# ShiLab-Bioinformatics/subread

Hardware: AMD Instinct MI355X
Metric: Mreads/s aligned, 100bp SE vs 3Gbp index; 1/2/4/8-GPU scaling + HBM GB/s (higher is better)
Workload: dtype u32; 1 GPU; C3: 50M x 100bp SE reads vs 3.0 Gbp 24-contig genome, full one-block index; read_len=100, mode=subread-align SE, parallelism=reads sharded across 1 GPU(s), index replicated, no collective

## Files before the change

### subread_amd/csrc/svg_device.h

```cpp
#ifndef SVG_DEVICE_H
#define SVG_DEVICE_H
#include <hip/hip_runtime.h>
#include <stdint.h>
#include "subread_vote.h"
#include "svg_internal.h"

struct DevIndex {
	const uint32_t *bstart;
	const int16_t *keys;
	const uint32_t *vals;
	const uint8_t *values;
	const uint32_t *chr_end;
	uint32_t nb, n_chr;
	uint32_t start_point, length, start_base_offset, values_bytes;
	int32_t gap, padding;
	const uint32_t *bgrp;
	const uint8_t *keys8;
	const uint4 *bline;
	const uint4 *bcode;
	const uint32_t *khash;
	const uint32_t *khash_ff;
	uint64_t khash_lines;
	int32_t khash_sec;
	const uint32_t *ksorted;
// ... 130 lines not shown
	return 0;
}

int svg_index_finish_device(svg_index *h);

static inline int svg_ensure(svg_index *h, void **p, size_t *cap, size_t need)
{
	if (need <= *cap) return 0;
	hipFree(*p);
	*p = NULL;
	*cap = 0;
	if (dmalloc(h, p, need)) return SVG_E_NOMEM;
	*cap = need;
	return 0;
}

void svg_io_free(svg_index *h);
void svg_long_ws_free(svg_index *h);

struct KParams {
	svg_params p;
	DevIndex ix;
	const char *seq1, *seq2;
	const uint64_t *off1, *off2;
	const uint16_t *len1, *len2;
	uint64_t n_reads;
	uint8_t *out;
	uint8_t *jout;
	uint16_t *bm_out;
	uint32_t *scratch;
	unsigned long long *stats;
	int tol, ii_end;
	uint32_t low, high;
	const uint2 *precs;
	int nps;
	uint32_t prec_stride;
	const uint32_t *idx;
	const uint32_t *idx_count;
	uint32_t *work;
	int32_t static_eighths;
	int stored;
	uint32_t *err;
};

struct PParams {
	DevIndex ix;
	const char *seq1, *seq2;
	const uint64_t *off1, *off2;
	const uint16_t *len1, *len2;
	uint32_t n_reads;
	int nps;
	int total_subreads, reverse_r1, reverse_r2;
	uint64_t nb_magic;
	uint2 *out;
	int soa;
	int window;
	int readmajor;
	unsigned long long *stats;
	uint32_t group;
	uint32_t *big_list, *big_count;
	uint32_t big_stride, big_regions;
	int packed;
	const uint32_t *pk_bases[2], *pk_xmask[2];
	const uint64_t *pk_starts[2];
	uint64_t pk_stride[2], pk_base0[2];
};

struct VoteJob {
	KParams kp;
	PParams pp;
	int npmax, nps, ends;
	bool sj, lane, overlap_mode;
	uint64_t per_read, chunk;
};
int svg_vote_prepare(svg_index *h, const svg_params *p, const svg_reads *r1, const svg_reads *r2, svg_mapping_result *out,
                     svg_subjunc_result *jout, uint16_t *big_margin, VoteJob *job);
int svg_vote_chunk(svg_index *h, VoteJob *job, uint64_t c0, uint64_t cn, int slot, hipStream_t st, hipStream_t st2);
int svg_vote_chunk_probe(svg_index *h, VoteJob *job, uint64_t c0, uint64_t cn, int slot, hipStream_t st);
int svg_vote_chunk_vote(svg_index *h, VoteJob *job, uint64_t c0, uint64_t cn, int slot, hipStream_t st, hipStream_t st2);
int svg_vote_batch_device_packed(svg_index *h, const svg_params *p, const svg_reads *r1, const svg_reads *r2,
                                 const svg_packed_reads *pk, svg_mapping_result *out, svg_subjunc_result *jout,
                                 uint16_t *big_margin, hipStream_t stream);

int svg_lane_eligible(const svg_index *h, const svg_params *p, int paired, int sj);
int svg_check_params(const svg_index *h, const svg_params *p, int paired);
int svg_lane_chunk(svg_index *h, int slot, const svg_params *p, const uint16_t *len, uint32_t n, const uint2 *precs,
                   int nps, uint8_t *out, uint8_t *jout, uint16_t *bm, const char *seq, const uint64_t *off,
                   unsigned long long *stats, uint32_t **defer_list, uint32_t **defer_count, hipStream_t st);
int svg_lane_pe_chunk(svg_index *h, int slot, const svg_params *p, const uint16_t *len1, const uint16_t *len2, uint32_t n,
                      const uint2 *precs, int nps, uint8_t *out, uint8_t *jout, uint16_t *bm_out, const char *seq1,
                      const uint64_t *off1, const char *seq2, const uint64_t *off2, unsigned long long *stats,
                      uint32_t **defer_list, uint32_t **defer_count, hipStream_t st);
int svg_timing_mark(svg_index *h, int k, int phase, hipStream_t st);

#endif
```

### subread_amd/csrc/svg_vote.hip

```cpp
#include <hip/hip_runtime.h>
#include <string>
#include <vector>
#include <chrono>
#include <atomic>
#include <deque>
#include <condition_variable>
#include <mutex>
#include <thread>
#include <pthread.h>
#include <sys/mman.h>
#include <stdint.h>
#include <string.h>
#include <stdlib.h>
#include <stdio.h>
#include "subread_vote.h"
#include "svg_internal.h"
#include "svg_device.h"

#define ROWS 30
#define SPACE 24
#define PSTR 25
#define NSLOT (ROWS * PSTR)
#define REC_LEN 21
#define COLD_WORDS 8
#define JCW 17

#define CAND_CAP 64
template <int ENDS, int MAXL, int MAXP, bool SJ>
struct WaveLDS {
	static constexpr int MAXS = ENDS == 1 ? 16 : 64;
	static constexpr int CAPL = ENDS == 2 ? 64 : 1;
	uint2 pm[NSLOT];
	uint2 cl[CAPL];
	uint16_t cls[CAPL];
	uint32_t pmid[ENDS][2][MAXP];
	uint16_t pfwd[ENDS][2][MAXP];
	uint16_t pbwd[ENDS][2][MAXP];
	uint32_t pcum[MAXP + 1];
	uint32_t res[ENDS][3][17];
	uint32_t tmp[ENDS][3][17];
	uint32_t jres[SJ ? ENDS : 1][3][4];
	uint32_t jtmp[SJ ? ENDS : 1][3][4];
	uint32_t simp_pos[ENDS][MAXS];
	uint16_t simp_slot[ENDS][MAXS];
	uint16_t simp_votes[ENDS][MAXS];
	int32_t simp_loc[ENDS == 2 ? 2 : 1][ENDS == 2 ? MAXS : 1];
	int16_t simp_chr[ENDS == 2 ? 2 : 1][ENDS == 2 ? MAXS : 1];
	uint16_t bm[SJ ? ENDS : 1][10];
	uint8_t rnew[32];
	alignas(16) unsigned long long btab[32];
	uint8_t gwin[SJ ? 2 : 1][SJ ? 64 : 4];
	char text[SJ ? ENDS : 1][2][SJ ? MAXL : 4];
};

__device__ __forceinline__ int lane_id() { return __lane_id(); }
__device__ __forceinline__ unsigned long long ballot(bool p) { return __ballot(p); }
__device__ __forceinline__ int lanes_below(unsigned long long m) { return __popcll(m & ((1ull << lane_id()) - 1ull)); }
__device__ __forceinline__ void wsync() { __builtin_amdgcn_fence(__ATOMIC_SEQ_CST, "wavefront"); __builtin_amdgcn_wave_barrier(); }
__device__ __forceinline__ int wave_max(int v)
{
	for (int o = 32; o; o >>= 1) { int t = __shfl_xor(v, o); v = t > v ? t : v; }
	return v;
}
__device__ __forceinline__ int wave_min(int v)
{
	for (int o = 32; o; o >>= 1) { int t = __shfl_xor(v, o); v = t < v ? t : v; }
	return v;
}
__device__ __forceinline__ uint32_t wave_sum(uint32_t v)
{
// ... 1296 lines not shown
	};
	auto uni = [](uint64_t v) -> uint64_t {
		return (uint64_t)(uint32_t)__builtin_amdgcn_readfirstlane((int)(uint32_t)v) |
		       ((uint64_t)(uint32_t)__builtin_amdgcn_readfirstlane((int)(uint32_t)(v >> 32)) << 32);
	};
	auto dyn_after = [&](uint64_t p) { return kp.idx && p + nw >= n_static; };
	uint64_t i = !kp.idx || gw < n_static ? gw : (n ? grab() : n);
	uint64_t in = i >= n ? n : (dyn_after(i) ? grab() : i + nw);
	uint64_t r = uni(i < n ? (kp.idx ? kp.idx[i] : i) : 0);
	if (i < n) { W.prefetch_text(r); W.prefetch_recs(r); }
	while (i < n) {
		const bool dyn = in < n && dyn_after(in);
		uint32_t nxt = 0;
		if (dyn && lane_id() == 0) nxt = atomicAdd(kp.work, 1u);
		const uint64_t rn = uni(in < n ? (kp.idx ? kp.idx[in] : in) : kp.n_reads);
		W.run_read(r, rn);
		const uint64_t in2 = in >= n ? n : (dyn ? n_static + (uint64_t)(uint32_t)__builtin_amdgcn_readfirstlane(__shfl((int)nxt, 0)) : in + nw);
		i = in;
		r = rn;
		in = in2;
#ifdef SVG_STAMPS
		{ unsigned long long _t = __builtin_amdgcn_s_memtime(); W.acc[5] += _t - W.t_last; W.t_last = _t; }
#endif
	}
#ifdef SVG_STAMPS
	if (kp.stats && lane_id() == 0) {
		for (int k = 0; k < 8; k++) atomicAdd(&kp.stats[8 + k], W.acc[k]);
		for (int k = 8; k < 12; k++) atomicAdd(&kp.stats[21 + k - 8], W.acc[k]);
		for (int k = 0; k < 4; k++) atomicAdd(&kp.stats[28 + k], W.why[k]);
	}
#endif
}

__device__ __forceinline__ bool try_run(uint64_t eq, int n, int &m, int &fwd, int &bwd, bool &hit)
{
	const int fe = eq ? __builtin_ctzll(eq) : 0, ne = __popcll(eq);
	if (eq && eq != (((ne == 64 ? 0ull : (1ull << ne)) - 1ull) << fe)) return false;
	if (eq) {
		const int le = fe + ne - 1;
		int lo = 0, hi = n - 1;
		for (;;) {
			m = (lo + hi) >> 1;
			if (m < fe) lo = m + 1;
			else if (m > le) hi = m - 1;
			else break;
		}
		hit = true;
		fwd = le - m + 1;
		bwd = m - fe;
	}
	return true;
}

template <int ENDS, bool PACKED>
__device__ __forceinline__ bool probe_key(const PParams &pp, uint32_t r, int e, int s, int p, uint32_t &key)
{
	int len = e ? pp.len2[r] : pp.len1[r];
	if (len > SVG_READ_KEEP) len = SVG_READ_KEEP;
	const int gap = pp.ix.gap;
	if (len < 15 + gap) return false;
	const int cr = (len - 15 - gap) << 16;
	int step;
	if (len <= 160) { step = cr / (pp.total_subreads - 1); if (step < (gap << 16)) step = gap << 16; }
	else { step = 6 << 16; if (cr / step > 62) step = cr / 62; }
	const int np = (1 + cr / step) * gap;
	if (p >= np) return false;
	const int k = p / gap, x = p - k * gap;
	int off = (int)(((int64_t)step * k) >> 16);
	if (gap > 1) off -= off % gap - x;
	const int rev = e ? pp.reverse_r2 : pp.reverse_r1;
	const bool direct = s == rev;
	const int start = direct ? off : len - 16 - off;
	key = 0;
	if constexpr (PACKED) {
		const uint64_t k0 = (pp.pk_starts[e] ? pp.pk_starts[e][r] : pp.pk_base0[e] + (uint64_t)r * pp.pk_stride[e]) +
		                    (uint64_t)start;
		const uint32_t *bw = pp.pk_bases[e] + (k0 >> 4);
		const uint32_t s2 = 2u * (uint32_t)(k0 & 15u);
		const uint32_t W = s2 ? (bw[0] << s2) | (bw[1] >> (32u - s2)) : bw[0];
		uint32_t X2 = 0;
		if (pp.pk_xmask[e]) {
			const uint32_t *xw = pp.pk_xmask[e] + (k0 >> 5);
			const uint32_t s1 = (uint32_t)(k0 & 31u);
			uint32_t t = (s1 > 16u ? (xw[0] << s1) | (xw[1] >> (32u - s1)) : xw[0] << s1) >> 16;
			t = (t | (t << 8)) & 0x00ff00ffu;
			t = (t | (t << 4)) & 0x0f0f0f0fu;
			t = (t | (t << 2)) & 0x33333333u;
			t = (t | (t << 1)) & 0x55555555u;
			X2 = t | (t << 1);
		}
		if (direct) key = (s == 1 && rev) ? (W | X2) : W;
		else {
			const uint32_t v = __builtin_bitreverse32(~W | X2);
			key = ((v >> 1) & 0x55555555u) | ((v & 0x55555555u) << 1);
		}
	} else {
		const char *src = (e ? pp.seq2 : pp.seq1) + (e ? pp.off2[r] : pp.off1[r]) + start;
		const uintptr_t a = (uintptr_t)src;
		const uint32_t *w = (const uint32_t *)(a & ~(uintptr_t)3);
		const int sh = (int)(a & 3);
		uint32_t wd[5];
#pragma unroll
		for (int q = 0; q < 4; q++) wd[q] = w[q];
		wd[4] = sh ? w[4] : 0u;
#pragma unroll
		for (int i = 0; i < 16; i++) {
			const int bi = sh + (direct ? i : 15 - i);
			char c = (char)((wd[bi >> 2] >> (8 * (bi & 3))) & 0xff);
			if (!direct) c = comp(c);
			if (s == 1 && rev) c = comp(comp(c));
			key |= b2i(c) << (30 - 2 * i);
		}
	}
	return true;
}

template <int ENDS, int BPC, bool LINE, bool PACKED>
__global__ void __launch_bounds__(256, BPC) probe_kernel(PParams pp)
{
	const DevIndex &ix = pp.ix;
	const uint32_t nps = (uint32_t)pp.nps, per_read = ENDS * 2 * nps;
	const uint32_t total = pp.n_reads * per_read;
	const int gap = ix.gap;
	unsigned long long st_p = 0, st_i = 0, st_h = 0;
	const uint32_t tiles = (total + 255u) / 256u, per_blk = (tiles + gridDim.x - 1u) / gridDim.x;
	const uint32_t tile_end = min(tiles, (blockIdx.x + 1u) * per_blk);
	for (uint32_t tile = blockIdx.x * per_blk; tile < tile_end; tile++) {
		const uint32_t t = tile * 256u + threadIdx.x;
		if (t >= total) break;
		uint32_t r, rem;
		if (pp.soa && !pp.readmajor) { rem = t / pp.n_reads; r = t - rem * pp.n_reads; }
		else { r = t / per_read; rem = t - r * per_read; }
		const int e = ENDS == 2 ? (int)(rem / (2 * nps)) : 0;
		const uint32_t rem2 = rem - (uint32_t)e * 2 * nps;
		const int s = rem2 >= nps ? 1 : 0;
		const int p = (int)(rem2 - (uint32_t)s * nps);
		uint2 rec = make_uint2(0u, 0u);
		uint32_t key;
		if (probe_key<ENDS, PACKED>(pp, r, e, s, p, key)) {
			{
				const uint32_t q = (uint32_t)__umul64hi((uint64_t)key, pp.nb_magic);
				const uint32_t b = key - q * ix.nb;
				const int16_t k16 = (int16_t)q;
				uint32_t first;
				int n;
				bool compact = false, inl = false;
				uint4 lw[4];
				if constexpr (LINE) {
					const uint4 *l4 = ix.bline + 4 * (size_t)b;
#pragma unroll
					for (int q = 0; q < 4; q++) lw[q] = l4[q];
					const uint32_t c = lw[0].y & 255u;
					first = lw[0].x;
					n = (int)c;
					compact = c != 255u;
					inl = c <= 59u;
				} else if (ix.bgrp) {
					const uint4 *g4 = (const uint4 *)(ix.bgrp + 8 * (size_t)(b >> 4));
					const uint4 ga = g4[0], gb = g4[1];
					const uint32_t i = b & 15u;
					const uint32_t cw[4] = {ga.y, ga.z, ga.w, gb.x};
					uint32_t pre = 0;
					bool sat = false;
#pragma unroll
					for (int q = 0; q < 4; q++) {
						const int nb_ = (int)i - 4 * q;
// ... 71 lines not shown
								const uint32_t x = dw[q] ^ kk;
								const uint32_t z = ~(((x & 0x7fff7fffu) + 0x7fff7fffu) | x | 0x7fff7fffu);
								const int j = 4 * k + q;
								eq |= ((uint64_t)((z >> 15) & 1u) << (2 * j)) | ((uint64_t)(z >> 31) << (2 * j + 1));
							}
						}
						eq = (eq >> sh) & ((1ull << n) - 1ull);
						done = try_run(eq, n, m, fwd, bwd, hit);
					}
					if (!done) {
						int lo = 0, hi = n - 1;
						for (;;) {
							m = (lo + hi) >> 1;
							int16_t kk = K[m];
							if (kk > k16) hi = m - 1;
							else if (kk < k16) lo = m + 1;
							else { hit = true; break; }
							if (hi < lo) break;
						}
						if (hit) {
							int qq = m + 1;
							while (qq < n && K[qq] == k16) qq++;
							fwd = qq - m;
							qq = m - 1;
							while (qq >= 0 && K[qq] == k16) qq--;
							bwd = m - 1 - qq;
						}
					}
					if (hit) {
						rec = make_uint2(first + (uint32_t)m, (uint32_t)fwd | ((uint32_t)bwd << 16));
						st_h += (unsigned)(fwd + bwd);
					}
				}
			}
		}
		pp.out[pp.soa ? (size_t)rem * pp.n_reads + r : (size_t)t] = rec;
	}
	if (pp.stats) {
		for (int o = 32; o; o >>= 1) {
			st_p += __shfl_xor(st_p, o); st_i += __shfl_xor(st_i, o); st_h += __shfl_xor(st_h, o);
		}
		if (lane_id() == 0 && st_p) {
			atomicAdd(&pp.stats[0], st_p);
			atomicAdd(&pp.stats[1], st_i);
			atomicAdd(&pp.stats[2], st_h);
		}
	}
}

#define PROBE_GROUP_RECS 2048
#define IMG_LINE  0
#define IMG_CODE  1
#define IMG_KHASH 2
template <int ENDS, bool PACKED>
struct ProbeDepth { static constexpr int value = 2; };

__device__ __forceinline__ void code_record(const uint4 u0, const uint4 u1, uint32_t q, uint32_t key, uint2 &rec, bool &big,
                                            unsigned long long &st_i, unsigned long long &st_h)
{
	const uint32_t c = u0.y & 255u, first = u0.x;
	big = c == 255u;
	if (!big && c) {
		const uint64_t z[4] = {~(((uint64_t)u0.y << 32) | u0.x) & ~0xffffffffffull, ~(((uint64_t)u0.w << 32) | u0.z),
		                       ~(((uint64_t)u1.y << 32) | u1.x), ~(((uint64_t)u1.w << 32) | u1.z)};
		const int k = (int)q;
		const int fe = k ? code_zero(z, k - 1) - 40 - (k - 1) : 0;
		const int ee = code_zero(z, k) - 40 - k;
		st_i += c;
		if (ee > fe) {
			const int le = ee - 1;
			int lo = 0, hi = (int)c - 1, m;
			for (;;) {
				m = (lo + hi) >> 1;
				if (m < fe) lo = m + 1;
				else if (m > le) hi = m - 1;
				else break;
			}
			rec = make_uint2(first + (uint32_t)m, (uint32_t)(le - m + 1) | ((uint32_t)(m - fe) << 16));
			st_h += (unsigned)(ee - fe);
		}
	}
	if (big) rec = make_uint2(key, 0xffffffffu);
}

template <int ENDS, bool PACKED, int IMG>
__global__ void __launch_bounds__(256, 8) probe_line_kernel(PParams pp)
{
	__shared__ uint2 srec[PROBE_GROUP_RECS];
	__shared__ uint32_t s_big;
	const DevIndex &ix = pp.ix;
	const uint32_t nps = (uint32_t)pp.nps, per_read = ENDS * 2 * nps, n = pp.n_reads, G = pp.group;
	const uint32_t ngroups = (n + G - 1) / G, per_blk = (ngroups + gridDim.x - 1) / gridDim.x;
	const uint32_t g_end = min(ngroups, (blockIdx.x + 1) * per_blk);
	uint32_t *const big_list = pp.big_list + (size_t)blockIdx.x * pp.big_stride;
	unsigned long long st_p = 0, st_i = 0, st_h = 0;
	if (threadIdx.x == 0) s_big = 0;
	__syncthreads();
	for (uint32_t g = blockIdx.x * per_blk; g < g_end; g++) {
		const uint32_t r0 = g * G, nr = min(G, n - r0), np = nr * per_read, npr = (np + 255u) & ~255u;
		if constexpr (IMG == IMG_CODE) for (uint32_t i0 = threadIdx.x; i0 < npr; i0 += 256u * ProbeDepth<ENDS, PACKED>::value) {
			uint32_t key[ProbeDepth<ENDS, PACKED>::value], outidx[ProbeDepth<ENDS, PACKED>::value], q[ProbeDepth<ENDS, PACKED>::value];
			bool ok[ProbeDepth<ENDS, PACKED>::value];
#pragma unroll
			for (int t = 0; t < ProbeDepth<ENDS, PACKED>::value; t++) {
				const uint32_t i = i0 + 256u * (uint32_t)t;
				key[t] = outidx[t] = q[t] = 0u;
				ok[t] = false;
				if (i < np) {
					const uint32_t rl = i / per_read, rem = i - rl * per_read, r = r0 + rl;
					const int e = ENDS == 2 ? (int)(rem / (2 * nps)) : 0;
					const uint32_t rem2 = rem - (uint32_t)e * 2 * nps;
					const int s = rem2 >= nps ? 1 : 0;
					const int p = (int)(rem2 - (uint32_t)s * nps);
					outidx[t] = pp.soa ? rem * n + r : r * per_read + rem;
					ok[t] = probe_key<ENDS, PACKED>(pp, r, e, s, p, key[t]);
				}
			}
			uint4 u0[ProbeDepth<ENDS, PACKED>::value], u1[ProbeDepth<ENDS, PACKED>::value];
#pragma unroll
			for (int t = 0; t < ProbeDepth<ENDS, PACKED>::value; t++) {
				u0[t] = u1[t] = make_uint4(0u, 0u, 0u, 0u);
				if (ok[t]) {
					q[t] = (uint32_t)__umul64hi((uint64_t)key[t], pp.nb_magic);
					const uint4 *c4 = ix.bcode + 2 * (size_t)(key[t] - q[t] * ix.nb);
					u0[t] = c4[0];
					u1[t] = c4[1];
				}
			}
#pragma unroll
			for (int t = 0; t < ProbeDepth<ENDS, PACKED>::value; t++) {
				const uint32_t i = i0 + 256u * (uint32_t)t;
				if (i - threadIdx.x >= npr) break;
				uint2 rec = make_uint2(0u, 0u);
				bool big = false;
				if (ok[t]) {
					st_p++;
					code_record(u0[t], u1[t], q[t], key[t], rec, big, st_i, st_h);
				}
				const unsigned long long bm = ballot(big);
				if (bm) {
					const int leader = __ffsll((long long)bm) - 1;
					uint32_t base = 0;
					if (lane_id() == leader) base = atomicAdd(&s_big, (uint32_t)__popcll(bm));
					base = __shfl(base, leader);
					if (big) big_list[base + lanes_below(bm)] = outidx[t];
				}
				if (i < np) srec[i] = rec;
			}
		}
		if (IMG == IMG_KHASH && ix.khash_sec) for (uint32_t i0 = threadIdx.x; i0 < npr; i0 += 256u * ProbeDepth<ENDS, PACKED>::value) {
			uint32_t key[ProbeDepth<ENDS, PACKED>::value], outidx[ProbeDepth<ENDS, PACKED>::value];
			uint64_t L[ProbeDepth<ENDS, PACKED>::value];
			bool ok[ProbeDepth<ENDS, PACKED>::value];
#pragma unroll
			for (int t = 0; t < ProbeDepth<ENDS, PACKED>::value; t++) {
				const uint32_t i = i0 + 256u * (uint32_t)t;
				key[t] = outidx[t] = 0u;
				L[t] = 0u;
				ok[t] = false;
				if (i < np) {
					const uint32_t rl = i / per_read, rem = i - rl * per_read, r = r0 + rl;
					const int e = ENDS == 2 ? (int)(rem / (2 * nps)) : 0;
					const uint32_t rem2 = rem - (uint32_t)e * 2 * nps;
					const int s = rem2 >= nps ? 1 : 0;
					const int p = (int)(rem2 - (uint32_t)s * nps);
					outidx[t] = pp.soa ? rem * n + r : r * per_read + rem;
					ok[t] = probe_key<ENDS, PACKED>(pp, r, e, s, p, key[t]);
				}
			}
			uint4 a[ProbeDepth<ENDS, PACKED>::value], b4[ProbeDepth<ENDS, PACKED>::value];
#pragma unroll
			for (int t = 0; t < ProbeDepth<ENDS, PACKED>::value; t++) {
				a[t] = b4[t] = make_uint4(0u, 0u, 0u, 0u);
				if (ok[t] && key[t] != 0xffffffffu) {
					L[t] = khash_line(key[t], ix.khash_lines);
					const uint4 *l4 = (const uint4 *)(ix.khash + 8 * L[t]);
					a[t] = l4[0];
					b4[t] = l4[1];
				}
			}
#pragma unroll
			for (int t = 0; t < ProbeDepth<ENDS, PACKED>::value; t++) {
				const uint32_t i = i0 + 256u * (uint32_t)t;
				if (i - threadIdx.x >= npr) break;
				uint2 rec = make_uint2(0u, 0u);
				if (ok[t]) {
					st_p++;
					if (pp.stats) {
						const uint32_t q = (uint32_t)__umul64hi((uint64_t)key[t], pp.nb_magic), b = key[t] - q * ix.nb;
						st_i += ix.bstart[b + 1] - ix.bstart[b];
					}
					if (key[t] == 0xffffffffu) khash_find(ix, key[t], rec);
					else {
						bool more;
						if (!khash_sector(a[t], b4[t], key[t], rec, more) && more)
							khash_find_from(ix, key[t], L[t] + 1 == ix.khash_lines ? 0 : L[t] + 1, rec);
					}
					if (pp.stats) st_h += (rec.y & 0xffffu) + (rec.y >> 16);
				}
				if (i < np) srec[i] = rec;
			}
		}
		if (IMG != IMG_CODE && !(IMG == IMG_KHASH && ix.khash_sec)) for (uint32_t i = threadIdx.x; i < npr; i += 256u) {
			uint2 rec = make_uint2(0u, 0u);
			bool big = false;
			uint32_t outidx = 0;
			if (i < np) {
				const uint32_t rl = i / per_read, rem = i - rl * per_read, r = r0 + rl;
				const int e = ENDS == 2 ? (int)(rem / (2 * nps)) : 0;
				const uint32_t rem2 = rem - (uint32_t)e * 2 * nps;
				const int s = rem2 >= nps ? 1 : 0;
				const int p = (int)(rem2 - (uint32_t)s * nps);
				outidx = pp.soa ? rem * n + r : r * per_read + rem;
				uint32_t key;
				if (IMG == IMG_KHASH && probe_key<ENDS, PACKED>(pp, r, e, s, p, key)) {
					st_p++;
					if (pp.stats) {
						const uint32_t q = (uint32_t)__umul64hi((uint64_t)key, pp.nb_magic), b = key - q * ix.nb;
						st_i += ix.bstart[b + 1] - ix.bstart[b];
					}
					khash_find(ix, key, rec);
					if (pp.stats) st_h += (rec.y & 0xffffu) + (rec.y >> 16);
				} else if (IMG == IMG_LINE && probe_key<ENDS, PACKED>(pp, r, e, s, p, key)) {
					const uint32_t q = (uint32_t)__umul64hi((uint64_t)key, pp.nb_magic);
					const uint32_t b = key - q * ix.nb;
					const uint4 *l4 = ix.bline + 4 * (size_t)b;
					uint4 lw[4];
#pragma unroll
					for (int k = 0; k < 4; k++) lw[k] = l4[k];
					const uint32_t c = lw[0].y & 255u, first = lw[0].x;
					st_p++;
					big = c > 59u;
					if (!big && c) {
						const uint32_t kk = (uint32_t)(uint8_t)q * 0x01010101u;
						uint64_t eq = 0;
#pragma unroll
						for (int k = 0; k < 4; k++) {
							const uint32_t dw[4] = {lw[k].x, lw[k].y, lw[k].z, lw[k].w};
#pragma unroll
							for (int qq = 0; qq < 4; qq++) {
								const uint32_t x = dw[qq] ^ kk;
								const uint32_t z = ~(((x & 0x7f7f7f7fu) + 0x7f7f7f7fu) | x | 0x7f7f7f7fu);
								const uint32_t bits = ((z >> 7) & 1u) | ((z >> 14) & 2u) | ((z >> 21) & 4u) | ((z >> 28) & 8u);
								eq |= (uint64_t)bits << (16 * k + 4 * qq);
							}
						}
						eq = (eq >> 5) & ((1ull << c) - 1ull);
						int m = 0, fwd = 0, bwd = 0;
						bool hit = false;
						if (try_run(eq, (int)c, m, fwd, bwd, hit)) {
							st_i += c;
							if (hit) {
								rec = make_uint2(first + (uint32_t)m, (uint32_t)fwd | ((uint32_t)bwd << 16));
								st_h += (unsigned)(fwd + bwd);
							}
						} else big = true;
					}
					if (big) rec = make_uint2(key, 0xffffffffu);
				}
			}
			const unsigned long long bm = ballot(big);
			if (bm) {
				const int leader = __ffsll((long long)bm) - 1;
				uint32_t base = 0;
				if (lane_id() == leader) base = atomicAdd(&s_big, (uint32_t)__popcll(bm));
				base = __shfl(base, leader);
				if (big) big_list[base + lanes_below(bm)] = outidx;
			}
			if (i < np) srec[i] = rec;
		}
		__syncthreads();
		for (uint32_t i = threadIdx.x; i < np; i += 256u) {
			if (pp.soa) {
				const uint32_t row = i / nr, rl = i - row * nr;
				pp.out[(size_t)row * n + r0 + rl] = srec[rl * per_read + row];
			} else pp.out[(size_t)r0 * per_read + i] = srec[i];
		}
		__syncthreads();
	}
	if (threadIdx.x == 0) pp.big_count[blockIdx.x] = s_big;
	if (pp.stats) {
		for (int o = 32; o; o >>= 1) {
			st_p += __shfl_xor(st_p, o); st_i += __shfl_xor(st_i, o); st_h += __shfl_xor(st_h, o);
		}
		if (lane_id() == 0 && st_p) {
			atomicAdd(&pp.stats[0], st_p);
			atomicAdd(&pp.stats[1], st_i);
			atomicAdd(&pp.stats[2], st_h);
		}
	}
}

__global__ void __launch_bounds__(256) probe_big_kernel(PParams pp)
{
	const DevIndex &ix = pp.ix;
	const int sub = (int)(threadIdx.x & 7u);
	unsigned long long st_i = 0, st_h = 0, st_n = 0;
	for (uint32_t reg = blockIdx.x; reg < pp.big_regions; reg += gridDim.x) {
		const uint32_t cnt = pp.big_count[reg];
		const uint32_t *list = pp.big_list + (size_t)reg * pp.big_stride;
		st_n += threadIdx.x == 0 ? cnt : 0u;
		for (uint32_t j = threadIdx.x >> 3; j < cnt; j += 32u) {
			const uint32_t outidx = list[j];
			const uint32_t key = pp.out[outidx].x;
			const uint32_t q = (uint32_t)__umul64hi((uint64_t)key, pp.nb_magic);
			const uint32_t b = key - q * ix.nb;
			const uint16_t k16 = (uint16_t)q;
			const uint2 l0 = ix.bcode ? *(const uint2 *)(ix.bcode + 2 * (size_t)b) : *(const uint2 *)(ix.bline + 4 * (size_t)b);
			const uint32_t first = l0.x;
			uint32_t nn = l0.y & 255u;
			if (nn == 255u) nn = ix.bstart[b + 1] - first;
			const int16_t *K = ix.keys + first;
			const uint4 *W = (const uint4 *)((uintptr_t)K & ~(uintptr_t)15);
			const int sh = (int)(((uintptr_t)K & 15) >> 1);
			const int nw = (sh + (int)nn + 7) >> 3;
			int fe = 0x7fffffff, le = -1, ne = 0;
			for (int w0 = 0; w0 < nw; w0 += 32) {
				uint4 v[4];
#pragma unroll
				for (int ps = 0; ps < 4; ps++) {
					const int w = w0 + 8 * ps + sub;
					v[ps] = w < nw ? W[w] : make_uint4(0xffffffffu, 0xffffffffu, 0xffffffffu, 0xffffffffu);
				}
#pragma unroll
				for (int ps = 0; ps < 4; ps++) {
					const int w = w0 + 8 * ps + sub;
					const uint32_t dw[4] = {v[ps].x, v[ps].y, v[ps].z, v[ps].w};
#pragma unroll
					for (int h = 0; h < 8; h++) {
						const int it = 8 * w + h - sh;
						if (it >= 0 && it < (int)nn && (uint16_t)(dw[h >> 1] >> (16 * (h & 1))) == k16) {
							fe = min(fe, it); le = max(le, it); ne++;
						}
					}
				}
			}
#pragma unroll
			for (int o = 4; o; o >>= 1) {
				fe = min(fe, __shfl_xor(fe, o));
				le = max(le, __shfl_xor(le, o));
				ne += __shfl_xor(ne, o);
// ... 1022 lines not shown
#ifndef SVG_SE_OCC
#define SVG_SE_OCC 7
#endif
	return npmax <= 32 ? launch_t<1, 256, 32, 2, SVG_SE_OCC, false>(h, kp, st) : launch_t<1, 256, 64, 2, SVG_SE_OCC, false>(h, kp, st);
}

int svg_vote_prepare(svg_index *h, const svg_params *p, const svg_reads *r1, const svg_reads *r2, svg_mapping_result *out,
                     svg_subjunc_result *jout, uint16_t *big_margin, VoteJob *job)
{
	if (!h || !p || !r1 || !out) { svg_set_error("svg_vote_batch_device: NULL argument"); return SVG_E_ARG; }
	if (r2 && r2->n_reads != r1->n_reads) { svg_set_error("R1/R2 read counts differ"); return SVG_E_ARG; }
	int rc = svg_check_params(h, p, r2 != NULL);
	if (rc) return rc;
	if (p->do_breakpoint_detection && !jout) { svg_set_error("do_breakpoint_detection needs jout"); return SVG_E_ARG; }
	if (p->do_big_margin_filtering_for_junctions && !big_margin) { svg_set_error("big-margin filtering needs big_margin"); return SVG_E_ARG; }
	KParams &kp = job->kp;
	memset(&kp, 0, sizeof kp);
	kp.err = h->d_err;
	kp.p = *p;
	kp.ix = h->dix;
	kp.seq1 = r1->seq; kp.off1 = r1->offsets; kp.len1 = r1->lens;
	if (r2) { kp.seq2 = r2->seq; kp.off2 = r2->offsets; kp.len2 = r2->lens; }
	kp.n_reads = r1->n_reads;
	kp.out = (uint8_t *)out;
	kp.jout = (uint8_t *)jout;
	kp.bm_out = big_margin;
	kp.tol = p->max_indel_length < 16 ? p->max_indel_length : 16;
	kp.ii_end = 5;
	if (kp.tol > 5) kp.ii_end = (kp.tol % 5) ? (kp.tol - kp.tol % 5 + 5) : kp.tol;
	kp.low = h->dix.start_base_offset;
	kp.high = h->dix.start_base_offset + h->dix.length;
	kp.stats = h->stats_on ? h->d_stats : NULL;
	job->npmax = svg_probe_bound(h->max_read_len, h->dix.gap, p->total_subreads);
	job->sj = p->do_breakpoint_detection || p->do_big_margin_filtering_for_junctions;
	if (job->npmax > 192) { svg_set_error("%d subreads per strand exceed 192", job->npmax); return SVG_E_UNSUPPORTED; }
	job->ends = r2 ? 2 : 1;
	const int nps = job->npmax > 0 ? job->npmax : 1;
	job->nps = nps;
	job->per_read = (uint64_t)job->ends * 2 * nps;
	uint64_t chunk = ((uint64_t)1 << 30) / (job->per_read * 8);
	if (chunk > (uint64_t)0x7fffffff / job->per_read) chunk = (uint64_t)0x7fffffff / job->per_read;
	{ const int64_t oc = svg_get_option("chunk"); if (oc > 0 && (uint64_t)oc < chunk) chunk = (uint64_t)oc; }
	if (chunk < 1) chunk = 1;
	job->chunk = chunk;
	const int64_t oo = svg_get_option("overlap");
	job->overlap_mode = oo >= 0 ? oo == 1 : (!job->sj && !r2);
	PParams &pp = job->pp;
	memset(&pp, 0, sizeof pp);
	pp.ix = h->dix;
	pp.seq1 = kp.seq1; pp.seq2 = kp.seq2;
	pp.nps = nps;
	pp.total_subreads = p->total_subreads; pp.reverse_r1 = p->reverse_r1; pp.reverse_r2 = p->reverse_r2;
	pp.nb_magic = ~0ull / h->dix.nb + 1;
	pp.stats = kp.stats;
	job->lane = svg_lane_eligible(h, p, r2 != NULL, job->sj) != 0 && (!r2 || nps <= (job->sj ? 14 : 10)) && (!job->sj || nps <= 14) &&
	            !h->stored;
	kp.stored = h->stored;
	pp.soa = job->lane ? 1 : 0;
	pp.window = h->dix.nb >= 131073u;
	pp.readmajor = 1;
	return 0;
}

int svg_vote_chunk(svg_index *h, VoteJob *job, uint64_t c0, uint64_t cn, int slot, hipStream_t st, hipStream_t st2)
{
	int rc = svg_vote_chunk_probe(h, job, c0, cn, slot, st);
	return rc ? rc : svg_vote_chunk_vote(h, job, c0, cn, slot, st, st2);
}

int svg_vote_chunk_probe(svg_index *h, VoteJob *job, uint64_t c0, uint64_t cn, int slot, hipStream_t st)
{
	if (slot < 0 || slot > 2) { svg_set_error("chunk slot %d out of range", slot); return SVG_E_ARG; }
	const KParams &kp = job->kp;
	int rc;
	if ((rc = svg_ensure(h, &h->d_prec[slot], &h->prec_cap[slot], cn * job->per_read * 8))) return rc;
	PParams pp = job->pp;
	pp.out = (uint2 *)h->d_prec[slot];
	pp.off1 = kp.off1 + c0; pp.len1 = kp.len1 + c0;
	if (kp.len2) { pp.off2 = kp.off2 + c0; pp.len2 = kp.len2 + c0; }
	pp.n_reads = (uint32_t)cn;
	uint64_t pb = (cn * job->per_read + 255) / 256, pmax = (uint64_t)h->n_cu * 32;
	if (pb > pmax) pb = pmax;
	if ((rc = timing_mark(h, 0, 0, st))) return rc;
	const bool pe = kp.len2 != NULL;
	if (pp.packed) {
		for (int e = 0; e < (pe ? 2 : 1); e++) {
			if (pp.pk_starts[e]) pp.pk_starts[e] += c0;
			else pp.pk_base0[e] += c0 * pp.pk_stride[e];
		}
	}
#define PROBE_LAUNCH(E, L, P) hipLaunchKernelGGL((probe_kernel<E, 8, L, P>), dim3((unsigned)pb), dim3(256), 0, st, pp)
	if (h->dix.bline || h->dix.bcode || h->dix.khash) {
		pp.group = (uint32_t)(PROBE_GROUP_RECS / job->per_read);
		if (pp.group > 64) pp.group = 64;
		if (pp.group < 1) pp.group = 1;
		const uint64_t ng = (cn + pp.group - 1) / pp.group;
		const int64_t pc = svg_get_option("probe_cap");
		uint64_t gb = ng, gmax = (uint64_t)h->n_cu * (pc > 0 ? (uint64_t)pc : 32u);
		if (gb > gmax) gb = gmax;
		const uint64_t per_blk = (ng + gb - 1) / gb, stride = per_blk * pp.group * job->per_read;
		const uint64_t cnt_words = (gb + 63) & ~63ull;
		if ((rc = svg_ensure(h, &h->d_big[slot], &h->big_cap[slot], (cnt_words + gb * stride) * 4 + 256))) return rc;
		pp.big_count = (uint32_t *)h->d_big[slot];
		pp.big_list = (uint32_t *)h->d_big[slot] + cnt_words;
		pp.big_stride = (uint32_t)stride;
		pp.big_regions = (uint32_t)gb;
#define LINE_LAUNCH(E, P, C) hipLaunchKernelGGL((probe_line_kernel<E, P, C>), dim3((unsigned)gb), dim3(256), 0, st, pp)
		if (h->dix.khash) {
			if (pp.packed) { if (pe) LINE_LAUNCH(2, true, IMG_KHASH); else LINE_LAUNCH(1, true, IMG_KHASH); }
			else { if (pe) LINE_LAUNCH(2, false, IMG_KHASH); else LINE_LAUNCH(1, false, IMG_KHASH); }
		} else if (h->dix.bcode) {
			if (pp.packed) { if (pe) LINE_LAUNCH(2, true, IMG_CODE); else LINE_LAUNCH(1, true, IMG_CODE); }
			else { if (pe) LINE_LAUNCH(2, false, IMG_CODE); else LINE_LAUNCH(1, false, IMG_CODE); }
		} else {
			if (pp.packed) { if (pe) LINE_LAUNCH(2, true, IMG_LINE); else LINE_LAUNCH(1, true, IMG_LINE); }
			else { if (pe) LINE_LAUNCH(2, false, IMG_LINE); else LINE_LAUNCH(1, false, IMG_LINE); }
		}
#undef LINE_LAUNCH
		HIPCHK(hipGetLastError());
		if (!h->dix.khash) hipLaunchKernelGGL(probe_big_kernel, dim3((unsigned)(h->n_cu * 8)), dim3(256), 0, st, pp);
	} else if (h->dix.bline) {
		if (pp.packed) { if (pe) PROBE_LAUNCH(2, true, true); else PROBE_LAUNCH(1, true, true); }
		else { if (pe) PROBE_LAUNCH(2, true, false); else PROBE_LAUNCH(1, true, false); }
	} else {
		if (pp.packed) { if (pe) PROBE_LAUNCH(2, false, true); else PROBE_LAUNCH(1, false, true); }
		else { if (pe) PROBE_LAUNCH(2, false, false); else PROBE_LAUNCH(1, false, false); }
	}
#undef PROBE_LAUNCH
	HIPCHK(hipGetLastError());
	return timing_mark(h, 0, 1, st);
}

int svg_vote_chunk_vote(svg_index *h, VoteJob *job, uint64_t c0, uint64_t cn, int slot, hipStream_t st, hipStream_t st2)
{
	const KParams &kp = job->kp;
	const svg_params *p = &kp.p;
	const int ends = job->ends, nps = job->nps;
	const bool pe = kp.len2 != NULL;
	int rc;
	h->wave_cap = 0;
	if (st2 != st) {
		const int64_t ow = svg_get_option("wave_cap");
		h->wave_cap = ow >= 0 ? (int)ow : SVG_WAVE_CAP;
	}
	KParams kc = kp;
	kc.off1 = kp.off1 + c0; kc.len1 = kp.len1 + c0;
	if (pe) { kc.off2 = kp.off2 + c0; kc.len2 = kp.len2 + c0; }
	kc.n_reads = cn;
// ... 145 lines not shown
```

Baseline: 549.9 Mreads/s.

## Precompute per-read probe plans in shared memory and restructure probe-line indexing

Each probe group now computes per-read plan data (base offset, clipped length, step, probe count) once into shared memory, and the group size is forced to a power of two. This replaces per-probe integer divisions and repeated length and offset loads with shifts, masks and a magic-number divide by gap. The record staging layout is changed to slot-major with a diagonal swizzle so both SoA and AoS write-outs stay conflict-light, and the code-image zero lookup reuses one select for both endpoints. Stats counters drop to 32-bit and are gated on a flag. A power-of-two group can be smaller than before, which lowers records per group and adds a sync per group.

```diff
diff --git a/subread_amd/csrc/svg_device.h b/subread_amd/csrc/svg_device.h
--- a/subread_amd/csrc/svg_device.h
+++ b/subread_amd/csrc/svg_device.h
@@ -206,6 +206,7 @@
 	int nps;
 	int total_subreads, reverse_r1, reverse_r2;
 	uint64_t nb_magic;
+	uint32_t gap_magic;
 	uint2 *out;
 	int soa;
 	int window;
diff --git a/subread_amd/csrc/svg_plan.h b/subread_amd/csrc/svg_plan.h
--- /dev/null
+++ b/subread_amd/csrc/svg_plan.h
@@ -0,0 +1,69 @@
+#ifndef SVG_PLAN_H
+#define SVG_PLAN_H
+#include <stdint.h>
+#include "subread_vote.h"
+
+#if defined(__HIPCC__)
+#define SVG_PLAN_FN __host__ __device__ __forceinline__
+#else
+#define SVG_PLAN_FN static inline
+#endif
+
+SVG_PLAN_FN int svg_plan_read(int len, int gap, int total_subreads, int *clen, int *step)
+{
+	if (len > SVG_READ_KEEP) len = SVG_READ_KEEP;
+	*clen = len;
+	*step = 0;
+	if (len < 15 + gap) return 0;
+	const int cr = (len - 15 - gap) << 16;
+	int st;
+	if (len <= 160) { st = cr / (total_subreads - 1); if (st < (gap << 16)) st = gap << 16; }
+	else { st = 6 << 16; if (cr / st > 62) st = cr / 62; }
+	*step = st;
+	return (1 + cr / st) * gap;
+}
+
+SVG_PLAN_FN uint32_t svg_plan_gap_magic(int gap) { return gap > 1 ? 0xffffffffu / (uint32_t)gap + 1u : 0u; }
+SVG_PLAN_FN uint32_t svg_plan_div_gap(uint32_t x, uint32_t magic) { return (uint32_t)(((uint64_t)x * magic) >> 32); }
+
+SVG_PLAN_FN int svg_plan_off(int step, int p, int gap, uint32_t magic)
+{
+	if (gap == 1) return (int)(uint32_t)(((uint64_t)(uint32_t)step * (uint32_t)p) >> 16);
+	const uint32_t k = svg_plan_div_gap((uint32_t)p, magic), x = (uint32_t)p - k * (uint32_t)gap;
+	const uint32_t off = (uint32_t)(((uint64_t)(uint32_t)step * k) >> 16);
+	return (int)(off - (off - svg_plan_div_gap(off, magic) * (uint32_t)gap) + x);
+}
+
+SVG_PLAN_FN void svg_plan_pack(uint64_t base, int len, int step, int np, uint32_t w[3])
+{
+	w[0] = (uint32_t)base;
+	w[1] = ((uint32_t)(base >> 32) & 0xffffu) | ((uint32_t)len << 16);
+	w[2] = ((uint32_t)step & 0xffffffu) | ((uint32_t)(np > 255 ? 255 : np) << 24);
+}
+SVG_PLAN_FN uint64_t svg_plan_base(const uint32_t w[3]) { return w[0] | ((uint64_t)(w[1] & 0xffffu) << 32); }
+SVG_PLAN_FN int svg_plan_len(const uint32_t w[3]) { return (int)(w[1] >> 16); }
+SVG_PLAN_FN int svg_plan_step(const uint32_t w[3]) { return (int)(w[2] & 0xffffffu); }
+SVG_PLAN_FN int svg_plan_np(const uint32_t w[3]) { return (int)(w[2] >> 24); }
+
+SVG_PLAN_FN uint32_t svg_plan_group_log2(uint32_t recs, uint32_t per_read)
+{
+	uint32_t g = recs / per_read, lg = 0;
+	if (g > 64u) g = 64u;
+	while ((2u << lg) <= g) lg++;
+	return lg;
+}
+
+template <int ENDS>
+SVG_PLAN_FN void svg_plan_index(uint32_t i, uint32_t lg, uint32_t nps, uint32_t *rl, uint32_t *slot, int *e, int *s, int *p)
+{
+	*rl = i & ((1u << lg) - 1u);
+	const uint32_t sl = i >> lg;
+	uint32_t es = sl >= nps ? 1u : 0u;
+	if (ENDS == 2) es += (sl >= 2u * nps ? 1u : 0u) + (sl >= 3u * nps ? 1u : 0u);
+	*slot = sl;
+	*e = (int)(es >> 1);
+	*s = (int)(es & 1u);
+	*p = (int)(sl - es * nps);
+}
+
+#endif
diff --git a/subread_amd/csrc/svg_vote.hip b/subread_amd/csrc/svg_vote.hip
--- a/subread_amd/csrc/svg_vote.hip
+++ b/subread_amd/csrc/svg_vote.hip
@@ -16,6 +16,7 @@
 #include "subread_vote.h"
 #include "svg_internal.h"
 #include "svg_device.h"
+#include "svg_plan.h"
 
 #define ROWS 30
 #define SPACE 24
@@ -1418,29 +1419,15 @@
 	return true;
 }
 
-template <int ENDS, bool PACKED>
-__device__ __forceinline__ bool probe_key(const PParams &pp, uint32_t r, int e, int s, int p, uint32_t &key)
-{
-	int len = e ? pp.len2[r] : pp.len1[r];
-	if (len > SVG_READ_KEEP) len = SVG_READ_KEEP;
-	const int gap = pp.ix.gap;
-	if (len < 15 + gap) return false;
-	const int cr = (len - 15 - gap) << 16;
-	int step;
-	if (len <= 160) { step = cr / (pp.total_subreads - 1); if (step < (gap << 16)) step = gap << 16; }
-	else { step = 6 << 16; if (cr / step > 62) step = cr / 62; }
-	const int np = (1 + cr / step) * gap;
-	if (p >= np) return false;
-	const int k = p / gap, x = p - k * gap;
-	int off = (int)(((int64_t)step * k) >> 16);
-	if (gap > 1) off -= off % gap - x;
+template <bool PACKED>
+__device__ __forceinline__ uint32_t probe_window(const PParams &pp, int e, int s, uint64_t base, int len, int off)
+{
 	const int rev = e ? pp.reverse_r2 : pp.reverse_r1;
 	const bool direct = s == rev;
 	const int start = direct ? off : len - 16 - off;
-	key = 0;
+	uint32_t key = 0;
 	if constexpr (PACKED) {
-		const uint64_t k0 = (pp.pk_starts[e] ? pp.pk_starts[e][r] : pp.pk_base0[e] + (uint64_t)r * pp.pk_stride[e]) +
-		                    (uint64_t)start;
+		const uint64_t k0 = base + (uint64_t)start;
 		const uint32_t *bw = pp.pk_bases[e] + (k0 >> 4);
 		const uint32_t s2 = 2u * (uint32_t)(k0 & 15u);
 		const uint32_t W = s2 ? (bw[0] << s2) | (bw[1] >> (32u - s2)) : bw[0];
@@ -1461,7 +1448,7 @@
 			key = ((v >> 1) & 0x55555555u) | ((v & 0x55555555u) << 1);
 		}
 	} else {
-		const char *src = (e ? pp.seq2 : pp.seq1) + (e ? pp.off2[r] : pp.off1[r]) + start;
+		const char *src = (e ? pp.seq2 : pp.seq1) + base + start;
 		const uintptr_t a = (uintptr_t)src;
 		const uint32_t *w = (const uint32_t *)(a & ~(uintptr_t)3);
 		const int sh = (int)(a & 3);
@@ -1478,6 +1465,23 @@
 			key |= b2i(c) << (30 - 2 * i);
 		}
 	}
+	return key;
+}
+
+template <bool PACKED>
+__device__ __forceinline__ uint64_t probe_read_base(const PParams &pp, uint32_t r, int e)
+{
+	if constexpr (PACKED) return pp.pk_starts[e] ? pp.pk_starts[e][r] : pp.pk_base0[e] + (uint64_t)r * pp.pk_stride[e];
+	else return e ? pp.off2[r] : pp.off1[r];
+}
+
+template <int ENDS, bool PACKED>
+__device__ __forceinline__ bool probe_key(const PParams &pp, uint32_t r, int e, int s, int p, uint32_t &key)
+{
+	int len, step;
+	const int gap = pp.ix.gap;
+	if (p >= svg_plan_read(e ? pp.len2[r] : pp.len1[r], gap, pp.total_subreads, &len, &step)) return false;
+	key = probe_window<PACKED>(pp, e, s, probe_read_base<PACKED>(pp, r, e), len, svg_plan_off(step, p, gap, pp.gap_magic));
 	return true;
 }
 
@@ -1655,21 +1659,37 @@
 #define IMG_LINE  0
 #define IMG_CODE  1
 #define IMG_KHASH 2
+#ifndef SVG_PROBE_DEPTH
+#define SVG_PROBE_DEPTH 2
+#endif
 template <int ENDS, bool PACKED>
-struct ProbeDepth { static constexpr int value = 2; };
+struct ProbeDepth { static constexpr int value = SVG_PROBE_DEPTH; };
 
 __device__ __forceinline__ void code_record(const uint4 u0, const uint4 u1, uint32_t q, uint32_t key, uint2 &rec, bool &big,
-                                            unsigned long long &st_i, unsigned long long &st_h)
+                                            uint32_t &items, uint32_t &hits)
 {
 	const uint32_t c = u0.y & 255u, first = u0.x;
 	big = c == 255u;
+	items = hits = 0u;
 	if (!big && c) {
 		const uint64_t z[4] = {~(((uint64_t)u0.y << 32) | u0.x) & ~0xffffffffffull, ~(((uint64_t)u0.w << 32) | u0.z),
 		                       ~(((uint64_t)u1.y << 32) | u1.x), ~(((uint64_t)u1.w << 32) | u1.z)};
 		const int k = (int)q;
-		const int fe = k ? code_zero(z, k - 1) - 40 - (k - 1) : 0;
-		const int ee = code_zero(z, k) - 40 - k;
-		st_i += c;
+		const int c0 = __popcll(z[0]), c1 = c0 + __popcll(z[1]), c2 = c1 + __popcll(z[2]);
+		const int j = k - 1;
+		const int w = (j >= c0 ? 1 : 0) + (j >= c1 ? 1 : 0) + (j >= c2 ? 1 : 0);
+		const uint64_t za = w == 0 ? z[0] : w == 1 ? z[1] : w == 2 ? z[2] : z[3];
+		const uint64_t zb = w == 0 ? z[1] : w == 1 ? z[2] : w == 2 ? z[3] : 0ull;
+		int fe = 0, pl = 39;
+		uint64_t wa = z[0], wb = z[1];
+		if (k) {
+			pl = select64(za, j - (w == 0 ? 0 : w == 1 ? c0 : w == 2 ? c1 : c2));
+			fe = 64 * w + pl - 40 - j;
+			wa = za; wb = zb;
+		}
+		const uint64_t win = (wa >> pl >> 1) | (wb << (63 - pl));
+		const int ee = win ? fe + __builtin_ctzll(win) : code_zero(z, k) - 40 - k;
+		items = c;
 		if (ee > fe) {
 			const int le = ee - 1;
 			int lo = 0, hi = (int)c - 1, m;
@@ -1680,44 +1700,79 @@
 				else break;
 			}
 			rec = make_uint2(first + (uint32_t)m, (uint32_t)(le - m + 1) | ((uint32_t)(m - fe) << 16));
-			st_h += (unsigned)(ee - fe);
+			hits = (uint32_t)(ee - fe);
 		}
 	}
 	if (big) rec = make_uint2(key, 0xffffffffu);
+}
+
+template <int ENDS, bool PACKED>
+__device__ __forceinline__ bool line_probe(const PParams &pp, const uint4 *splan, uint32_t i, uint32_t lg, uint32_t nr, uint32_t &key)
+{
+	uint32_t rl, slot;
+	int e, s, p;
+	svg_plan_index<ENDS>(i, lg, (uint32_t)pp.nps, &rl, &slot, &e, &s, &p);
+	if (rl >= nr) return false;
+	const uint4 pl = splan[((uint32_t)e << lg) + rl];
+	const uint32_t w[3] = {pl.x, pl.y, pl.z};
+	if (p >= svg_plan_np(w)) return false;
+	key = probe_window<PACKED>(pp, e, s, svg_plan_base(w), svg_plan_len(w), svg_plan_off(svg_plan_step(w), p, pp.ix.gap, pp.gap_magic));
+	return true;
+}
+
+__device__ __forceinline__ uint32_t line_stage(const PParams &pp, uint32_t i, uint32_t lg)
+{
+	const uint32_t m = (1u << lg) - 1u;
+	return pp.soa ? i : (i & ~m) | ((i + (i >> lg)) & m);
+}
+
+template <int ENDS>
+__device__ __forceinline__ uint32_t line_outidx(const PParams &pp, uint32_t i, uint32_t lg, uint32_t r0)
+{
+	const uint32_t r = r0 + (i & ((1u << lg) - 1u)), slot = i >> lg;
+	return pp.soa ? slot * pp.n_reads + r : r * (ENDS * 2u * (uint32_t)pp.nps) + slot;
 }
 
 template <int ENDS, bool PACKED, int IMG>
 __global__ void __launch_bounds__(256, 8) probe_line_kernel(PParams pp)
 {
 	__shared__ uint2 srec[PROBE_GROUP_RECS];
+	__shared__ uint4 splan[ENDS * 64];
 	__shared__ uint32_t s_big;
 	const DevIndex &ix = pp.ix;
-	const uint32_t nps = (uint32_t)pp.nps, per_read = ENDS * 2 * nps, n = pp.n_reads, G = pp.group;
-	const uint32_t ngroups = (n + G - 1) / G, per_blk = (ngroups + gridDim.x - 1) / gridDim.x;
+	const uint32_t nps = (uint32_t)pp.nps, per_read = ENDS * 2 * nps, n = pp.n_reads, G = pp.group, lg = 31u - (uint32_t)__clz(G);
+	const uint32_t ngroups = (n + G - 1) >> lg, per_blk = (ngroups + gridDim.x - 1) / gridDim.x;
 	const uint32_t g_end = min(ngroups, (blockIdx.x + 1) * per_blk);
 	uint32_t *const big_list = pp.big_list + (size_t)blockIdx.x * pp.big_stride;
-	unsigned long long st_p = 0, st_i = 0, st_h = 0;
+	const bool stats = pp.stats != nullptr;
+	uint32_t st_p = 0, st_i = 0, st_h = 0;
 	if (threadIdx.x == 0) s_big = 0;
 	__syncthreads();
 	for (uint32_t g = blockIdx.x * per_blk; g < g_end; g++) {
-		const uint32_t r0 = g * G, nr = min(G, n - r0), np = nr * per_read, npr = (np + 255u) & ~255u;
+		const uint32_t r0 = g << lg, nr = min(G, n - r0), np = per_read << lg, npr = (np + 255u) & ~255u;
+		if (threadIdx.x < ((uint32_t)ENDS << lg)) {
+			const uint32_t rl = threadIdx.x & (G - 1u);
+			const int e = (int)(threadIdx.x >> lg);
+			uint4 pl = make_uint4(0u, 0u, 0u, 0u);
+			if (rl < nr) {
+				const uint32_t r = r0 + rl;
+				int len, step;
+				const int nprobe = svg_plan_read(e ? pp.len2[r] : pp.len1[r], ix.gap, pp.total_subreads, &len, &step);
+				uint32_t w[3];
+				svg_plan_pack(probe_read_base<PACKED>(pp, r, e), len, step, nprobe, w);
+				pl = make_uint4(w[0], w[1], w[2], 0u);
+			}
+			splan[threadIdx.x] = pl;
+		}
+		__syncthreads();
 		if constexpr (IMG == IMG_CODE) for (uint32_t i0 = threadIdx.x; i0 < npr; i0 += 256u * ProbeDepth<ENDS, PACKED>::value) {
-			uint32_t key[ProbeDepth<ENDS, PACKED>::value], outidx[ProbeDepth<ENDS, PACKED>::value], q[ProbeDepth<ENDS, PACKED>::value];
+			uint32_t key[ProbeDepth<ENDS, PACKED>::value], q[ProbeDepth<ENDS, PACKED>::value];
 			bool ok[ProbeDepth<ENDS, PACKED>::value];
 #pragma unroll
 			for (int t = 0; t < ProbeDepth<ENDS, PACKED>::value; t++) {
 				const uint32_t i = i0 + 256u * (uint32_t)t;
-				key[t] = outidx[t] = q[t] = 0u;
-				ok[t] = false;
-				if (i < np) {
-					const uint32_t rl = i / per_read, rem = i - rl * per_read, r = r0 + rl;
-					const int e = ENDS == 2 ? (int)(rem / (2 * nps)) : 0;
-					const uint32_t rem2 = rem - (uint32_t)e * 2 * nps;
-					const int s = rem2 >= nps ? 1 : 0;
-					const int p = (int)(rem2 - (uint32_t)s * nps);
-					outidx[t] = pp.soa ? rem * n + r : r * per_read + rem;
-					ok[t] = probe_key<ENDS, PACKED>(pp, r, e, s, p, key[t]);
-				}
+				key[t] = q[t] = 0u;
+				ok[t] = i < np && line_probe<ENDS, PACKED>(pp, splan, i, lg, nr, key[t]);
 			}
 			uint4 u0[ProbeDepth<ENDS, PACKED>::value], u1[ProbeDepth<ENDS, PACKED>::value];
 #pragma unroll
@@ -1737,8 +1792,9 @@
 				uint2 rec = make_uint2(0u, 0u);
 				bool big = false;
 				if (ok[t]) {
-					st_p++;
-					code_record(u0[t], u1[t], q[t], key[t], rec, big, st_i, st_h);
+					uint32_t items, hits;
+					code_record(u0[t], u1[t], q[t], key[t], rec, big, items, hits);
+					if (stats) { st_p++; st_i += items; st_h += hits; }
 				}
 				const unsigned long long bm = ballot(big);
 				if (bm) {
@@ -1746,30 +1802,21 @@
 					uint32_t base = 0;
 					if (lane_id() == leader) base = atomicAdd(&s_big, (uint32_t)__popcll(bm));
 					base = __shfl(base, leader);
-					if (big) big_list[base + lanes_below(bm)] = outidx[t];
-				}
-				if (i < np) srec[i] = rec;
+					if (big) big_list[base + lanes_below(bm)] = line_outidx<ENDS>(pp, i, lg, r0);
+				}
+				if (i < np) srec[line_stage(pp, i, lg)] = rec;
 			}
 		}
 		if (IMG == IMG_KHASH && ix.khash_sec) for (uint32_t i0 = threadIdx.x; i0 < npr; i0 += 256u * ProbeDepth<ENDS, PACKED>::value) {
-			uint32_t key[ProbeDepth<ENDS, PACKED>::value], outidx[ProbeDepth<ENDS, PACKED>::value];
+			uint32_t key[ProbeDepth<ENDS, PACKED>::value];
 			uint64_t L[ProbeDepth<ENDS, PACKED>::value];
 			bool ok[ProbeDepth<ENDS, PACKED>::value];
 #pragma unroll
 			for (int t = 0; t < ProbeDepth<ENDS, PACKED>::value; t++) {
 				const uint32_t i = i0 + 256u * (uint32_t)t;
-				key[t] = outidx[t] = 0u;
+				key[t] = 0u;
 				L[t] = 0u;
-				ok[t] = false;
-				if (i < np) {
-					const uint32_t rl = i / per_read, rem = i - rl * per_read, r = r0 + rl;
-					const int e = ENDS == 2 ? (int)(rem / (2 * nps)) : 0;
-					const uint32_t rem2 = rem - (uint32_t)e * 2 * nps;
-					const int s = rem2 >= nps ? 1 : 0;
-					const int p = (int)(rem2 - (uint32_t)s * nps);
-					outidx[t] = pp.soa ? rem * n + r : r * per_read + rem;
-					ok[t] = probe_key<ENDS, PACKED>(pp, r, e, s, p, key[t]);
-				}
+				ok[t] = i < np && line_probe<ENDS, PACKED>(pp, splan, i, lg, nr, key[t]);
 			}
 			uint4 a[ProbeDepth<ENDS, PACKED>::value], b4[ProbeDepth<ENDS, PACKED>::value];
 #pragma unroll
@@ -1788,9 +1835,9 @@
 				if (i - threadIdx.x >= npr) break;
 				uint2 rec = make_uint2(0u, 0u);
 				if (ok[t]) {
-					st_p++;
-					if (pp.stats) {
+					if (stats) {
 						const uint32_t q = (uint32_t)__umul64hi((uint64_t)key[t], pp.nb_magic), b = key[t] - q * ix.nb;
+						st_p++;
 						st_i += ix.bstart[b + 1] - ix.bstart[b];
 					}
 					if (key[t] == 0xffffffffu) khash_find(ix, key[t], rec);
@@ -1799,32 +1846,25 @@
 						if (!khash_sector(a[t], b4[t], key[t], rec, more) && more)
 							khash_find_from(ix, key[t], L[t] + 1 == ix.khash_lines ? 0 : L[t] + 1, rec);
 					}
-					if (pp.stats) st_h += (rec.y & 0xffffu) + (rec.y >> 16);
-				}
-				if (i < np) srec[i] = rec;
+					if (stats) st_h += (rec.y & 0xffffu) + (rec.y >> 16);
+				}
+				if (i < np) srec[line_stage(pp, i, lg)] = rec;
 			}
 		}
 		if (IMG != IMG_CODE && !(IMG == IMG_KHASH && ix.khash_sec)) for (uint32_t i = threadIdx.x; i < npr; i += 256u) {
 			uint2 rec = make_uint2(0u, 0u);
 			bool big = false;
-			uint32_t outidx = 0;
-			if (i < np) {
-				const uint32_t rl = i / per_read, rem = i - rl * per_read, r = r0 + rl;
-				const int e = ENDS == 2 ? (int)(rem / (2 * nps)) : 0;
-				const uint32_t rem2 = rem - (uint32_t)e * 2 * nps;
-				const int s = rem2 >= nps ? 1 : 0;
-				const int p = (int)(rem2 - (uint32_t)s * nps);
-				outidx = pp.soa ? rem * n + r : r * per_read + rem;
-				uint32_t key;
-				if (IMG == IMG_KHASH && probe_key<ENDS, PACKED>(pp, r, e, s, p, key)) {
-					st_p++;
-					if (pp.stats) {
+			uint32_t key = 0;
+			if (i < np && line_probe<ENDS, PACKED>(pp, splan, i, lg, nr, key)) {
+				if (IMG == IMG_KHASH) {
+					if (stats) {
 						const uint32_t q = (uint32_t)__umul64hi((uint64_t)key, pp.nb_magic), b = key - q * ix.nb;
+						st_p++;
 						st_i += ix.bstart[b + 1] - ix.bstart[b];
 					}
 					khash_find(ix, key, rec);
-					if (pp.stats) st_h += (rec.y & 0xffffu) + (rec.y >> 16);
-				} else if (IMG == IMG_LINE && probe_key<ENDS, PACKED>(pp, r, e, s, p, key)) {
+					if (stats) st_h += (rec.y & 0xffffu) + (rec.y >> 16);
+				} else if (IMG == IMG_LINE) {
 					const uint32_t q = (uint32_t)__umul64hi((uint64_t)key, pp.nb_magic);
 					const uint32_t b = key - q * ix.nb;
 					const uint4 *l4 = ix.bline + 4 * (size_t)b;
@@ -1832,7 +1872,7 @@
 #pragma unroll
 					for (int k = 0; k < 4; k++) lw[k] = l4[k];
 					const uint32_t c = lw[0].y & 255u, first = lw[0].x;
-					st_p++;
+					if (stats) st_p++;
 					big = c > 59u;
 					if (!big && c) {
 						const uint32_t kk = (uint32_t)(uint8_t)q * 0x01010101u;
@@ -1852,10 +1892,10 @@
 						int m = 0, fwd = 0, bwd = 0;
 						bool hit = false;
 						if (try_run(eq, (int)c, m, fwd, bwd, hit)) {
-							st_i += c;
+							if (stats) st_i += c;
 							if (hit) {
 								rec = make_uint2(first + (uint32_t)m, (uint32_t)fwd | ((uint32_t)bwd << 16));
-								st_h += (unsigned)(fwd + bwd);
+								if (stats) st_h += (uint32_t)(fwd + bwd);
 							}
 						} else big = true;
 					}
@@ -1868,28 +1908,33 @@
 				uint32_t base = 0;
 				if (lane_id() == leader) base = atomicAdd(&s_big, (uint32_t)__popcll(bm));
 				base = __shfl(base, leader);
-				if (big) big_list[base + lanes_below(bm)] = outidx;
-			}
-			if (i < np) srec[i] = rec;
+				if (big) big_list[base + lanes_below(bm)] = line_outidx<ENDS>(pp, i, lg, r0);
+			}
+			if (i < np) srec[line_stage(pp, i, lg)] = rec;
 		}
 		__syncthreads();
-		for (uint32_t i = threadIdx.x; i < np; i += 256u) {
-			if (pp.soa) {
-				const uint32_t row = i / nr, rl = i - row * nr;
-				pp.out[(size_t)row * n + r0 + rl] = srec[rl * per_read + row];
-			} else pp.out[(size_t)r0 * per_read + i] = srec[i];
+		if (pp.soa) {
+			for (uint32_t i = threadIdx.x; i < np; i += 256u) {
+				const uint32_t rl = i & (G - 1u);
+				if (rl < nr) pp.out[(size_t)(i >> lg) * n + r0 + rl] = srec[i];
+			}
+		} else {
+			for (uint32_t rl = threadIdx.x >> 6; rl < nr; rl += 4u)
+				for (uint32_t slot = threadIdx.x & 63u; slot < per_read; slot += 64u)
+					pp.out[(size_t)(r0 + rl) * per_read + slot] = srec[(slot << lg) | ((rl + slot) & (G - 1u))];
 		}
 		__syncthreads();
 	}
 	if (threadIdx.x == 0) pp.big_count[blockIdx.x] = s_big;
-	if (pp.stats) {
+	if (stats) {
+		unsigned long long sp = st_p, si = st_i, sh = st_h;
 		for (int o = 32; o; o >>= 1) {
-			st_p += __shfl_xor(st_p, o); st_i += __shfl_xor(st_i, o); st_h += __shfl_xor(st_h, o);
-		}
-		if (lane_id() == 0 && st_p) {
-			atomicAdd(&pp.stats[0], st_p);
-			atomicAdd(&pp.stats[1], st_i);
-			atomicAdd(&pp.stats[2], st_h);
+			sp += __shfl_xor(sp, o); si += __shfl_xor(si, o); sh += __shfl_xor(sh, o);
+		}
+		if (lane_id() == 0 && sp) {
+			atomicAdd(&pp.stats[0], sp);
+			atomicAdd(&pp.stats[1], si);
+			atomicAdd(&pp.stats[2], sh);
 		}
 	}
 }
@@ -3018,6 +3063,7 @@
 	pp.nps = nps;
 	pp.total_subreads = p->total_subreads; pp.reverse_r1 = p->reverse_r1; pp.reverse_r2 = p->reverse_r2;
 	pp.nb_magic = ~0ull / h->dix.nb + 1;
+	pp.gap_magic = svg_plan_gap_magic(h->dix.gap);
 	pp.stats = kp.stats;
 	job->lane = svg_lane_eligible(h, p, r2 != NULL, job->sj) != 0 && (!r2 || nps <= (job->sj ? 14 : 10)) && (!job->sj || nps <= 14) &&
 	            !h->stored;
@@ -3057,9 +3103,7 @@
 	}
 #define PROBE_LAUNCH(E, L, P) hipLaunchKernelGGL((probe_kernel<E, 8, L, P>), dim3((unsigned)pb), dim3(256), 0, st, pp)
 	if (h->dix.bline || h->dix.bcode || h->dix.khash) {
-		pp.group = (uint32_t)(PROBE_GROUP_RECS / job->per_read);
-		if (pp.group > 64) pp.group = 64;
-		if (pp.group < 1) pp.group = 1;
+		pp.group = 1u << svg_plan_group_log2(PROBE_GROUP_RECS, (uint32_t)job->per_read);
 		const uint64_t ng = (cn + pp.group - 1) / pp.group;
 		const int64_t pc = svg_get_option("probe_cap");
 		uint64_t gb = ng, gmax = (uint64_t)h->n_cu * (pc > 0 ? (uint64_t)pc : 32u);
```

Measured after the change: 569.1 Mreads/s, median of 6. 3.5% higher.
